# eggeek/distributed-oracle-search

Measured on AMD Instinct MI355X. Metric: CPD build sources/sec + GTEPS; table-search queries/sec; % HBM roofline, higher is better.
Workload: dtype u32

## Files before the change

distributed-oracle-search_amd/cpd.py:

```python
from __future__ import annotations

import ctypes as C
import os

import numpy as np

_HERE = os.path.dirname(os.path.abspath(__file__))
LIB_PATH = os.environ.get("CPD_LIB") or os.path.join(_HERE, "libcpd.so")

CPD_OK = 0
CPD_E_ARG = -1
CPD_E_HIP = -2
CPD_E_OOM = -3
CPD_E_NOROW = -4
CPD_E_RANGE = -5
CPD_E_IO = -6
PART_DIV = 0
PART_MOD = 1
INF = 0xFFFFFFFF
FM_ALL = 0xFFFF
MAX_WEIGHT_SETS = 8
MAX_LOAD_SLICES = 8
LOADS_ACCUMULATE = 1
TIMED_LOADS = 2
# ... 9 lines not shown
    "cpd_debug_rows", "cpd_index_create", "cpd_index_from_rows", "cpd_index_set_weights",
    "cpd_query_batch", "cpd_query_prepare", "cpd_query_run", "cpd_query_fetch",
    "cpd_index_free", "cpd_timing_enable", "cpd_timing_reset", "cpd_timing_get",
    "cpd_index_set_mode", "cpd_index_get_mode", "cpd_plan_cache", "cpd_index_create_empty",
    "cpd_index_append_rows", "cpd_index_append_built_rows", "cpd_index_info",
    "cpd_synth_road_graph_ex", "cpd_query_search", "cpd_query_search_counters",
    "cpd_graph_set_coords", "cpd_host_alloc", "cpd_host_free",
    "cpd_rows_lanes", "cpd_graph_hint_next", "cpd_graph_set_hbm_reserve",
    "cpd_device_mem_info", "cpd_rows_move_words", "cpd_rows_export_moves",
    "cpd_index_append_moves", "cpd_device_arena", "cpd_device_arena_release", "cpd_batch_bytes",
    "cpd_rows_move_bits", "cpd_graph_move_bits", "cpd_bucket_bytes", "cpd_space_check",
    "cpd_query_paths", "cpd_query_paths_fetch", "cpd_query_search_paths",
    "cpd_index_set_weight_sets", "cpd_query_costs", "cpd_query_costs_fetch",
    "cpd_query_loads", "cpd_query_loads_fetch", "cpd_query_loads_clear", "cpd_query_search_loads",
    "cpd_query_timed", "cpd_query_timed_fetch",
]
SYNTH_STYLES = {"shuffled": 7, "spec": 0}
INDEX_MODES = {"auto": 0, "rle": 1, "dense": 2}
SEARCH_FORMS = {"auto": 0, "tables": 1, "walks": 2}


class CpdError(RuntimeError):
    def __init__(self, code: int, msg: str):
        super().__init__(f"libcpd error {code}: {msg}")
        self.code = code


class PlanOpts(C.Structure):
    _fields_ = [("threads", C.c_int), ("witness_settle", C.c_uint32), ("verbose", C.c_int),
                ("no_hierarchy", C.c_int), ("ch_gpu", C.c_int), ("ch_device", C.c_int)]
# ... 153 lines not shown


class RoadGraph:

    def __init__(self, row_ptr, dst, w, x=None, y=None):
        self.row_ptr, self.dst, self.w = _u32(row_ptr), _u32(dst), _u32(w)
        self.x, self.y = x, y

    @property
    def n(self) -> int:
        return len(self.row_ptr) - 1

    @property
    def m(self) -> int:
        return len(self.dst)


def synth_road_graph(width: int, height: int, seed: int, mean_outdeg: float = 2.5,
                     style: str = "shuffled") -> RoadGraph:
    flags = SYNTH_STYLES[style]
    n, m = C.c_uint32(), C.c_uint32()
    _check(lib.cpd_synth_road_graph_ex(width, height, C.c_double(mean_outdeg), C.c_uint64(seed),
                                       C.c_uint32(flags), C.byref(n), C.byref(m), None, None,
                                       None, None, None))
    rp = np.empty(n.value + 1, np.uint32)
    dst = np.empty(m.value, np.uint32)
    w = np.empty(m.value, np.uint32)
    x = np.empty(n.value, np.int32)
    y = np.empty(n.value, np.int32)
    _check(lib.cpd_synth_road_graph_ex(width, height, C.c_double(mean_outdeg), C.c_uint64(seed),
# ... 190 lines not shown

    def move_bits(self) -> int:
        b = C.c_uint32()
        _check(lib.cpd_graph_move_bits(self._h, C.byref(b)))
        return b.value

    def set_coords(self, x, y) -> None:
        if x is None or y is None:
            _check(lib.cpd_graph_set_coords(self._h, None, None))
            return
        xs = np.ascontiguousarray(x, dtype=np.int32)
        ys = np.ascontiguousarray(y, dtype=np.int32)
        if len(xs) != self.plan.info()["n"] or len(ys) != len(xs):
            raise ValueError("coordinates must have one entry per node")
        _check(lib.cpd_graph_set_coords(self._h, _ptr(xs, i32p), _ptr(ys, i32p)))

    def build_rows(self, targets, reuse: Rows | None = None) -> Rows:
        t = _u32(targets)
        h = C.c_void_p()
        _check(lib.cpd_build_rows(self._h, _ptr(t, u32p), C.c_uint32(len(t)),
                                  reuse._h if reuse else None, C.byref(h)))
        if reuse is not None:
            return reuse
        return Rows(h)

    def hint_next(self, targets) -> None:
        t = _u32(targets)
        _check(lib.cpd_graph_hint_next(self._h, _ptr(t, u32p), C.c_uint32(len(t))))

    def debug_rows(self, targets, want_dist=True, want_fm=True):
# ... 363 lines not shown
```

distributed-oracle-search_amd/csrc/cpd_gpu_internal.hpp:

```cpp
#pragma once
#include <hip/hip_runtime_api.h>

#include <algorithm>
#include <array>
#include <cstring>
#include <functional>
#include <map>
#include <memory>
#include <mutex>
#include <string>
#include <vector>

#include "cpd_internal.hpp"
#include "cpd_kernels.hpp"
#include "cpd_switches.hpp"

#define HIP_CHECK(expr)                                                          \
    do {                                                                         \
        hipError_t _e = (expr);                                                  \
        if (_e != hipSuccess)                                                    \
            throw ::cpd::Error(_e == hipErrorOutOfMemory ? CPD_E_OOM : CPD_E_HIP, \
                               std::string(#expr) + ": " + hipGetErrorString(_e)); \
    } while (0)

namespace cpd {

struct ArenaScope {
    ArenaScope();
    ~ArenaScope();
    ArenaScope(const ArenaScope&) = delete;
// ... 131 lines not shown
    uint32_t acquire_set() {
        const uint32_t x = cur;
        cur = (cur + 1u) % nsets;
        if (emit_pending[x]) {
            HIP_CHECK(hipStreamWaitEvent(stream, ev_emit[x], 0));
            emit_pending[x] = false;
        }
        return x;
    }
    void drain_emits() {
        if (estream) HIP_CHECK(hipStreamSynchronize(estream));
        for (auto& p : emit_pending) p = false;
    }
    bool leaf_fm = false;
    DevBuf<uint32_t> leafbits;
    DevBuf<uint16_t> fmleaf;
    bool narrow = false;
    static constexpr uint32_t kNarrowProbe = 2;
    uint32_t narrow_probe = kNarrowProbe;
    HostBuf<uint32_t> ovf_hb;
    uint32_t ovf_h() const { return ovf_hb.p ? ovf_hb.p[0] : 0u; }
    DevBuf<uint16_t> d16;
    DevBuf<uint32_t> dbase, ovf, pool;
    uint32_t pool_cap = 0;
    NarrowRows narrow_rows(bool on) {
        if (!on) return NarrowRows{nullptr, nullptr, n, nullptr, nullptr, 0};
        return NarrowRows{d16.p, dbase.p, n, ovf.p, pool.p, pool_cap};
    }
    double n_leaf = 0, m_leaf = 0;
    std::vector<double> dsc_lvl_leaves;
// ... 17 lines not shown
    hipStream_t ustream = nullptr;
    hipEvent_t ev_up = nullptr, ev_down = nullptr, ev_fm[2] = {nullptr, nullptr};
    bool prepped = false;
    uint32_t prep_slot = 0;
    std::vector<uint32_t> prep_targets, hint;
    void drop_prep() {
        if (ustream) HIP_CHECK(hipStreamSynchronize(ustream));
        prepped = false;
    }
    DevBuf<uint32_t> asc_lvl_of, dsc_lvl_of;
    std::vector<uint32_t> up_item_first;
    DevBuf<uint32_t> up_items, up_init_slots;
    uint32_t n_init_slots = 0;
    std::vector<uint32_t> lane_key;
    DevBuf<uint32_t> seg_order;
    bool timing = false;
    std::vector<hipEvent_t> ev_pool;
    std::vector<Pending> pending;
    std::map<std::string, Agg> agg;

    ~cpd_graph();

    hipEvent_t get_event() {
        if (ev_pool.empty()) {
            hipEvent_t e;
            HIP_CHECK(hipEventCreate(&e));
            return e;
        }
        hipEvent_t e = ev_pool.back();
        ev_pool.pop_back();
// ... 190 lines not shown
```

distributed-oracle-search_amd/csrc/cpd_graph.cpp:

```cpp
#include <cmath>
#include <thread>

#include "cpd_gpu_internal.hpp"

namespace {

uint64_t pool_rows(uint32_t n, uint32_t B) {
    return std::max<uint64_t>((uint64_t)n * (B / 256u) / 8u, 4ull * n);
}

double batch_bytes_per_row(uint32_t n, uint32_t n_up, uint32_t npad, uint32_t fmb, bool narrow,
                           bool leaf_fm, uint32_t mbits) {
    const double rle = rle_fused(fmb) ? 12.0 * rle_emit_chunks(npad)
                                      : 3.0 * 5.0 / 32.0 * npad +
                                            (fmb == 4 ? 12.0 * rle_count_chunks(npad) : 0.0);
    const double fin = narrow ? (2.0 + 4.0 / 256.0 + 0.5) * n : 4.0 * n;
    return fin + 8.0 * n_up + 3.0 * fmb / 8.0 * npad + rle + (leaf_fm ? 0.5 * n : 0.0) +
           2.0 * mbits / 8.0 * npad;
}

std::vector<uint32_t> level_order(const cpd_plan& p, const std::vector<uint32_t>& level,
                                  uint32_t nlev, std::vector<uint32_t>& lvl_first) {
    const uint32_t n = p.n;
    std::vector<uint32_t> cnt(nlev + 1, 0);
// ... 179 lines not shown
        g.bytes += p.bytes;
        for (auto& f : p.late) g.bytes += f();
        ev_pool.push_back(p.a);
        ev_pool.push_back(p.b);
    }
    pending.swap(keep);
}

void cpd_graph::reserve_batch(uint32_t want) {
    ArenaScope carve;
    if (want == 0) {
        size_t free_b = 0, total_b = 0;
        HIP_CHECK(hipMemGetInfo(&free_b, &total_b));
        const double per = batch_bytes_per_row(n, n_up, npad, fmb, narrow, leaf_fm,
                                               1u << tlb);
        const double fixed = narrow ? 4096.0 * n : 0.0;
        const double avail = free_b > hbm_reserve + fixed ? (double)free_b - hbm_reserve - fixed
                                                          : 0.0;
        const double fit = 0.85 * avail / per;
        CPD_REQUIRE(hbm_reserve == 0 || fit >= 1024.0, CPD_E_OOM,
                    "HBM reserve of " + std::to_string(hbm_reserve >> 20) + " MiB leaves " +
                        std::to_string((size_t)avail >> 20) + " MiB: too little for a 1024-row batch");
        want = (uint32_t)std::min((double)switches().batch_max, std::max(1024.0, std::floor(fit / 1024) * 1024));
    }
    want = (want + 1023u) / 1024u * 1024u;
    if (want == B && upx[0].p) return;
    drain_emits();
    drop_prep();
    B = want;
    for (int s = 0; s < 2; ++s) {
        upx[s].alloc(std::max<size_t>((size_t)n_up * B, 1));
// ... 227 lines not shown
    g->dsc_desc.upload(desc.data(), desc.size(), g->stream);
}

void mark_leaves(cpd_graph* g, const cpd_plan* p) {
    std::vector<uint32_t> lb(g->npad / 32u, 0u);
    g->dsc_lvl_leaves.assign(g->dsc_lvl.size(), 0.0);
    for (uint32_t v = 0; v < g->n; ++v)
        if (p->ch.level_up[v] == 0) {
            const uint32_t c = p->order[v];
            lb[c >> 5] |= 1u << (c & 31u);
            g->n_leaf += 1;
            g->m_leaf += p->row_ptr[v + 1] - p->row_ptr[v];
            g->dsc_lvl_leaves[p->ch.level_dn[v]] += 1;
        }
    g->leafbits.upload(lb.data(), lb.size(), g->stream);
}

void chunk_narrow_up_levels(cpd_graph* g) {
    constexpr uint32_t kNarrow = 1024u;
    const uint32_t C = sweep_chunk_arcs();
    std::vector<uint32_t> items, slots;
    g->up_item_first.assign(g->asc_lvl.size(), 0);
    for (size_t l = 0; l + 1 < g->asc_lvl.size(); ++l) {
        g->up_item_first[l] = (uint32_t)(items.size() / 4);
        const uint32_t s0 = g->asc_lvl[l], s1 = g->asc_lvl[l + 1];
        if (l < 2 || s1 - s0 > kNarrow) continue;
        for (uint32_t x = s0; x < s1; ++x) {
            slots.push_back(x);
            for (uint32_t a = g->asc_off_host[x]; a < g->asc_off_host[x + 1]; a += C)
                items.insert(items.end(),
// ... 22 lines not shown

}

extern "C" {

int cpd_batch_bytes(uint32_t n, uint32_t max_degree, uint32_t batch, uint64_t* bytes) {
    return guarded([&] {
        CPD_REQUIRE(bytes && batch % 1024u == 0 && batch > 0, CPD_E_ARG,
                    "batch_bytes: batch must be a positive multiple of 1024");
        uint32_t shift = 0;
        while ((1u << shift) < std::max(1u, max_degree)) ++shift;
        const uint32_t fmb = fm_bits(shift);
        const uint32_t npad = (n + kFmTile - 1u) / kFmTile * kFmTile;
        const uint32_t mbits = max_degree <= 2u ? 1u : max_degree <= 4u ? 2u : 4u;
        *bytes = (uint64_t)(batch_bytes_per_row(n, n, npad, fmb, true, fmb == 4, mbits) * batch) +
                 (uint64_t)batch * (n / 256u + 1u) * 4u + 4096ull * n + 512ull * n + (64ull << 20);
    });
}

int cpd_graph_create(const cpd_plan* p, int device, cpd_graph** out) {
    return guarded([&] {
        CPD_REQUIRE(p && out, CPD_E_ARG, "graph: null argument");
        *out = nullptr;
        require_device();
        const double tg0 = now_seconds();
        auto g = std::make_unique<cpd_graph>();
        g->device = device;
        g->select();
        create_streams(g.get());
        trace_step("streams", tg0);
        column_space_csr(g.get(), p);
// ... 33 lines not shown
        g->reserve_batch(batch);
    });
}

int cpd_graph_set_hbm_reserve(cpd_graph* g, uint64_t bytes) {
    return guarded([&] {
        CPD_REQUIRE(g, CPD_E_ARG, "null graph");
        g->hbm_reserve = bytes;
    });
}

int cpd_graph_set_coords(cpd_graph* g, const int32_t* x, const int32_t* y) {
    return guarded([&] {
        CPD_REQUIRE(g, CPD_E_ARG, "null graph");
        if (!x || !y) {
            g->lane_key.clear();
            g->seg_order.release();
            return;
        }
        g->lane_key = hilbert_keys(x, y, g->n);
        if (switches().fm_order) {
            const uint32_t nseg = g->npad / 32u;
            std::vector<uint32_t> node_of(g->n);
            for (uint32_t v = 0; v < g->n; ++v) node_of[g->order[v]] = v;
            std::vector<uint64_t> kv(nseg);
            for (uint32_t sg = 0; sg < nseg; ++sg) {
                const uint32_t c = std::min(g->n - 1u, sg * 32u + 16u);
                kv[sg] = ((uint64_t)g->lane_key[node_of[c]] << 32) | sg;
            }
            std::sort(kv.begin(), kv.end());
            std::vector<uint32_t> so(nseg);
            for (uint32_t i = 0; i < nseg; ++i) so[i] = (uint32_t)kv[i];
            g->select();
            g->seg_order.upload(so.data(), nseg, g->stream);
            HIP_CHECK(hipStreamSynchronize(g->stream));
        }
    });
}

int cpd_graph_move_bits(const cpd_graph* g, uint32_t* bits) {
    return guarded([&] {
        CPD_REQUIRE(g && bits, CPD_E_ARG, "null argument");
        *bits = g->move_bits;
    });
}

int cpd_graph_get_batch(const cpd_graph* g, uint32_t* batch) {
    return guarded([&] {
        CPD_REQUIRE(g && batch, CPD_E_ARG, "null argument");
        *batch = g->B;
    });
// ... 46 lines not shown
```

distributed-oracle-search_amd/csrc/cpd_kernels.hip:

```cpp
#include <hip/hip_ext.h>
#include <hip/hip_runtime.h>
#include <hipcub/hipcub.hpp>
#include <algorithm>
#include <cstdint>
#include <type_traits>

#include "cpd_kernels.hpp"
#include "cpd_switches.hpp"

namespace cpd {
namespace kern {

constexpr uint32_t INF = 0xFFFFFFFFu;
constexpr uint32_t kNoEdge = 0xFFFFFFFFu;

__device__ __forceinline__ uint32_t sat_add(uint32_t d, uint32_t w) {
    uint32_t s = d + w;
    return (s < d) ? INF : s;
}

#ifndef CPD_RLE_LOOKBACK
#define CPD_RLE_LOOKBACK 16
#endif
constexpr uint32_t kSeg = 32;
// ... 858 lines not shown
    for (int cg = 0; cg < NC; cg += G) {
        if (cg + G < NC) issue(nxt, cg + G);
        finish(cur, cg);
        if ((cg + G) % 8 == 0) {
            const int wi = (cg + G) / 8 - 1;
#pragma unroll
            for (int i = 0; i < 4; ++i) fm_stage[(threadIdx.x * 4u + (uint32_t)i) * 4u + wi] = pk[i][wi];
        }
        cur = nxt;
    }
    uint4* __restrict__ o = reinterpret_cast<uint4*>(fm) + fm4_piece(4u * l4, nseg, cb / kSeg);
    const uint4* st = reinterpret_cast<const uint4*>(fm_stage) + threadIdx.x * 4u;
#pragma unroll
    for (int i = 0; i < 4; ++i) o[i] = st[i];
    }
}

template <int FMB>
__device__ __forceinline__ void seg_pass(const uint32_t (&v)[FmFmt<FMB>::kWords], uint32_t c0,
                                         uint32_t& h, uint32_t& S, uint32_t& cnt) {
    using F = FmFmt<FMB>;
#pragma unroll
    for (int k = 0; k < 32; ++k) {
        const uint32_t f = (v[k / F::kPer] >> (FMB * (k % F::kPer))) & F::kAll;
        const bool brk = (S & f) == 0u;
        cnt += brk ? 1u : 0u;
        h = brk ? c0 + (uint32_t)k : h;
        S = brk ? f : (S & f);
    }
}
// ... 3340 lines not shown
    switch (shift) {
        case 0: launch(kern::first_moves<1, 4, NARROW>, grid, blk, s, adj, dist, tgt, B, n, npad, r, fm, leafbits, fmleaf, nr); break;
        case 1: launch(kern::first_moves<2, 2, NARROW>, grid, blk, s, adj, dist, tgt, B, n, npad, r, fm, leafbits, fmleaf, nr); break;
        case 2:
            if constexpr (!NARROW) launch(kern::first_moves<4, 2, false>, grid, blk, s, adj, dist, tgt, B, n, npad, r, fm, leafbits, fmleaf, nr);
            break;
        case 3: launch(kern::first_moves<8, 1, NARROW>, grid, blk, s, adj, dist, tgt, B, n, npad, r, fm, leafbits, fmleaf, nr); break;
        default: launch(kern::first_moves<16, 1, NARROW>, grid, blk, s, adj, dist, tgt, B, n, npad, r, fm, leafbits, fmleaf, nr); break;
    }
}

void launch_first_moves(const uint32_t* adj32, uint32_t shift, const uint32_t* dist,
                        const uint32_t* tgt, uint32_t B, uint32_t rows, uint32_t n,
                        uint32_t npad, uint32_t* fm, const uint32_t* leafbits,
                        const uint16_t* fmleaf, NarrowRows nr, hipStream_t s,
                        const uint32_t* seg_order) {
    constexpr uint32_t tpb = 64u * kFmWpb;
    const dim3 grid((npad / kern::kSeg) * ((rows + 1023u) / 1024u) * (256u / tpb)), blk(tpb);
    const uint2* adj = reinterpret_cast<const uint2*>(adj32);
    if (nr.d16 && shift == 2)
        launch_shm(kern::first_moves_n4<2>, dim3(grid.x / kFmSpw), blk, 64u * tpb, s, adj, dist,
                   tgt, B, n, npad, xcd_remap(), fm, leafbits, fmleaf, nr, seg_order, kFmSpw);
    else if (nr.d16)
        launch_first_moves_t<true>(adj, shift, dist, tgt, B, n, npad, fm, leafbits, fmleaf, nr,
                                   grid, blk, s);
    else
        launch_first_moves_t<false>(adj, shift, dist, tgt, B, n, npad, fm, leafbits, fmleaf, nr,
                                    grid, blk, s);
}

bool first_moves_reads_own(uint32_t shift, bool narrow) {
    return !(narrow && shift == 2);
}

void launch_rle_count(const uint32_t* fm, uint32_t fmb, uint32_t npad, uint32_t nrows,
// ... 627 lines not shown
```

distributed-oracle-search_amd/csrc/cpd_kernels.hpp:

```cpp
#pragma once
#include <hip/hip_runtime_api.h>
#include <cstdint>

namespace cpd {

void set_launch_events(hipEvent_t start, hipEvent_t stop);

struct NarrowRows {
    uint16_t* d16;
    uint32_t* base;
    uint32_t n;
    uint32_t* ovf;
    uint32_t* pool;
    uint32_t cap;
};


constexpr uint32_t kLeafBit = 0x80000000u;
constexpr uint32_t kL1Bit = 0x40000000u;

void launch_sweep(bool ascend, const uint32_t* nodes, const uint32_t* arc_off,
                  const uint32_t* arcs , uint32_t slot0,
                  uint32_t count, uint32_t* dist, uint32_t* up, uint32_t ubase,
                  const uint32_t* uidx, const uint32_t* tgt, uint32_t B, uint32_t slabs,
// ... 11 lines not shown
                            const uint32_t* tgt, uint32_t B, uint32_t slabs,
                            const uint32_t* asc_nodes, const uint32_t* asc_off,
                            const uint32_t* asc_arcs, uint32_t* live, const uint32_t* tmask,
                            hipStream_t s);
uint32_t sweep_chunk_arcs();

void launch_target_mask(const uint32_t* tgt, uint32_t B, uint32_t* tmask, hipStream_t s);

void launch_live_stats(bool ascend, const uint32_t* nodes, const uint32_t* arc_off,
                       const uint32_t* arcs, const uint32_t* lvl_of, uint32_t slot0,
                       uint32_t slot1, uint32_t ubase, const uint32_t* uidx,
                       const uint32_t* live, unsigned int* stat, hipStream_t s);

uint32_t fm_bits(uint32_t shift);

void launch_first_moves(const uint32_t* adj, uint32_t shift, const uint32_t* dist,
                        const uint32_t* tgt, uint32_t B, uint32_t rows, uint32_t n,
                        uint32_t npad, uint32_t* fm, const uint32_t* leafbits,
                        const uint16_t* fmleaf, NarrowRows nr, hipStream_t s,
                        const uint32_t* seg_order = nullptr);
bool first_moves_reads_own(uint32_t shift, bool narrow);

constexpr uint32_t kFmTile = 2048;

void launch_rle_count(const uint32_t* fm, uint32_t fmb, uint32_t npad, uint32_t nrows,
                      uint32_t* counts, uint32_t* st, uint8_t* rc, hipStream_t s,
                      const uint32_t* gate = nullptr);

void launch_rle_moves(const uint32_t* fm, uint32_t fmb, uint32_t npad, uint32_t nrows,
                      const uint32_t* st, const uint8_t* rc, const uint32_t* out_row,
                      uint32_t lb, uint32_t* dense, hipStream_t s);
uint32_t rle_emit_chunks(uint32_t npad);
void launch_rle_emit(const uint32_t* fm, uint32_t npad, uint32_t nrows, const uint32_t* out_row,
                     uint32_t lb, uint32_t* dense, uint32_t* xe, uint32_t* xs, uint32_t* cc,
                     uint32_t* counts, hipStream_t s);
// ... 161 lines not shown
```

distributed-oracle-search_amd/csrc/cpd_rows.cpp:

```cpp
#include "cpd_gpu_internal.hpp"

void cpd_rows::settle() const {
    std::lock_guard<std::mutex> l(settle_mu);
    HIP_CHECK(hipSetDevice(device));
    wait();
    for (auto& b : retired) spare.push_back(std::move(b));
    retired.clear();
    if (pending.empty()) return;
    for (auto& b : pending) {
        for (uint32_t i = 0; i < b->k; ++i)
            offsets.push_back(offsets.back() + b->counts.p[b->pos_of[i]]);
        spare.push_back(std::move(b));
    }
    pending.clear();
    total = offsets.back();
    hipStream_t st = thread_stream(device);
    off.upload(offsets.data(), offsets.size(), st);
    HIP_CHECK(hipStreamSynchronize(st));
}

cpd_rows::Batch* cpd_rows::new_batch(uint32_t B) {
    for (size_t i = 0; i < retired.size();) {
        if (hipEventQuery(retired[i]->ev) == hipSuccess) {
            spare.push_back(std::move(retired[i]));
// ... 162 lines not shown

void launch_fm(cpd_graph* g, uint32_t k, bool narrow, uint32_t* fm, uint32_t slot) {
    const uint32_t B = g->B, n = g->n;
    const NarrowRows nr = g->narrow_rows(narrow);
    const double drow = narrow ? 2.0 + 4.0 / 256.0 : 4.0;
    const uint32_t fslabs = (k + 1023u) / 1024u;
    const double nl = g->leaf_fm ? g->n_leaf : 0.0, ml = g->leaf_fm ? g->m_leaf : 0.0;
    const double own = first_moves_reads_own(g->adj_shift, narrow) ? drow * (n - nl) : 0.0;
    double fbytes =
        (own + drow * (g->m - ml) + 0.5 * nl + g->fmb / 8.0 * g->npad) *
            (fslabs * 1024.0) +
        8.0 * (double)(n - nl) * (double)(1u << g->adj_shift) * fslabs + 4.0 * g->npad / 32.0;
    g->timed("first_moves", fbytes, [&] {
        launch_first_moves(g->adj.p, g->adj_shift, g->dist.p, g->fm_tgt.p, B, k, n, g->npad,
                           fm, g->leaf_fm ? g->leafbits.p : nullptr,
                           g->leaf_fm ? g->fmleaf.p : nullptr, nr, g->stream, g->seg_order.p);
    });
    HIP_CHECK(hipEventRecord(g->ev_fm[slot], g->stream));
}

void launch_down_fm(cpd_graph* g, uint32_t k, bool narrow, uint32_t* fm, uint32_t slot) {
    launch_down(g, k, narrow, slot);
    launch_fm(g, k, narrow, fm, slot);
}

void prepare_targets(cpd_graph* g, const uint32_t* targets, uint32_t k, uint32_t slot) {
    auto& S = g->bs[slot];
    CPD_REQUIRE(g->has_ch, CPD_E_ARG,
                "graph was created from a plan without hierarchy: it can serve queries "
                "but not build rows");
    std::vector<uint32_t> cols(g->B), idx(k);
// ... 491 lines not shown
```

distributed-oracle-search_amd/csrc/cpd_switches.cpp:

```cpp
#include "cpd_switches.hpp"

#include <algorithm>
#include <cstdio>
#include <cstdlib>

namespace cpd {
namespace {

bool env_on(const char* name) {
    const char* e = std::getenv(name);
    return !(e && *e == '0');
}
bool env_set(const char* name) {
    const char* e = std::getenv(name);
    return e && *e && *e != '0';
}

Switches read_switches() {
    Switches s;
    s.live = env_on("CPD_LIVE");
    s.sort = env_on("CPD_SORT");
    s.lane_key = env_on("CPD_LANE_KEY");
    s.xcd = env_on("CPD_XCD");
    s.async = env_on("CPD_ASYNC");
// ... 6 lines not shown
    s.batch_max = (uint32_t)std::max(1024ul, std::min(32768ul, b / 1024ul * 1024ul));
    s.trace = env_set("CPD_TRACE");
    s.search_trace = env_set("CPD_SEARCH_TRACE");
    return s;
}

}

const Switches& switches() {
    static const Switches s = read_switches();
    return s;
}

bool narrow_rows_on() { return env_on("CPD_NARROW"); }

uint64_t search_pool_words(uint64_t words) {
    const char* e = std::getenv("CPD_SEARCH_POOL_WORDS");
    return e && *e ? std::min<uint64_t>(words, std::strtoull(e, nullptr, 10)) : words;
}

ChPrio ch_prio() {
    ChPrio p;
    if (const char* e = std::getenv("CPD_CH_PRIO")) {
        long a, b, c;
        if (std::sscanf(e, "%ld,%ld,%ld", &a, &b, &c) == 3) p = {a, b, c};
    }
    return p;
}

}
// ... 1 lines not shown
```

distributed-oracle-search_amd/csrc/cpd_switches.hpp:

```cpp
#pragma once
#include <cstdint>

namespace cpd {

struct Switches {
    bool live;
    bool sort;
    bool lane_key;
    bool xcd;
    bool async;
    bool rle_fused;
    bool leaffm;
    bool overlap;
    bool fm_order;
    uint32_t batch_max;
    bool trace;
    bool search_trace;
};
const Switches& switches();

bool narrow_rows_on();

uint64_t search_pool_words(uint64_t words);

struct ChPrio {
    int64_t ed = 8, deleted = 2, depth = 12;
};
ChPrio ch_prio();

}
```

include/cpd_api.h:

```cpp
#ifndef CPD_API_H
#define CPD_API_H

#include <stdint.h>
#include <stddef.h>

#ifdef __cplusplus
extern "C" {
#endif

#define CPD_OK          0
#define CPD_E_ARG      -1
#define CPD_E_HIP      -2
#define CPD_E_OOM      -3
#define CPD_E_NOROW    -4
#define CPD_E_RANGE    -5
#define CPD_E_IO       -6

#define CPD_PART_DIV    0
#define CPD_PART_MOD    1

#define CPD_MAX_DEGREE 15u
#define CPD_INF        0xFFFFFFFFu
#define CPD_FM_ALL     0xFFFFu

// ... 67 lines not shown
                    const uint32_t* w, uint32_t n, uint32_t m, const cpd_plan_opts* opts,
                    cpd_plan** out, int* status);
void cpd_plan_free(cpd_plan* p);

int  cpd_device_count(int* count);
int  cpd_device_mem_info(int device, uint64_t* free_bytes, uint64_t* total_bytes);
int  cpd_device_arena(int device, uint64_t bytes, int touch);
int  cpd_device_arena_release(int device);
int  cpd_batch_bytes(uint32_t n, uint32_t max_degree, uint32_t batch, uint64_t* bytes);
int  cpd_graph_create(const cpd_plan* p, int device, cpd_graph** out);
int  cpd_graph_set_batch(cpd_graph* g, uint32_t batch);
int  cpd_graph_get_batch(const cpd_graph* g, uint32_t* batch);
int  cpd_graph_move_bits(const cpd_graph* g, uint32_t* bits);
int  cpd_graph_set_hbm_reserve(cpd_graph* g, uint64_t bytes);
int  cpd_graph_set_coords(cpd_graph* g, const int32_t* x, const int32_t* y);
void cpd_graph_free(cpd_graph* g);

int  cpd_build_rows(cpd_graph* g, const uint32_t* targets, uint32_t ntargets,
                    cpd_rows* reuse, cpd_rows** out);
int  cpd_graph_hint_next(cpd_graph* g, const uint32_t* targets, uint32_t ntargets);
int  cpd_rows_count(const cpd_rows* r, uint32_t* nrows, uint64_t* total_runs);
int  cpd_rows_export(const cpd_rows* r, uint64_t* offsets ,
                     uint32_t* runs );
int  cpd_rows_export_range(const cpd_rows* r, uint32_t first, uint32_t count,
                           uint64_t* offsets , uint32_t* runs);
int  cpd_rows_move_words(const cpd_rows* r, uint32_t* words);
int  cpd_rows_move_bits(const cpd_rows* r, uint32_t* bits);
int  cpd_rows_export_moves(const cpd_rows* r, uint32_t first, uint32_t count,
                           uint32_t* moves );
int  cpd_rows_targets(const cpd_rows* r, uint32_t* targets );
// ... 147 lines not shown
```

Before: 443,000.

## Stage shared neighbour distance rows in LDS via precomputed first-move patch plans

Adds a host-built patch plan that groups spatially ordered 32-column segments into patches whose distinct neighbour rows fit in LDS. A new first-moves kernel loads those rows, the edge weights, index tables and leaf first-moves into LDS once per patch and strip, then computes argmin first moves from LDS. The aim is to avoid re-reading the same neighbour distance rows from HBM for every column. In exchange it costs host-side plan construction, extra device memory for plan tables and large LDS use per workgroup, which limits occupancy. It only runs on the narrow, coordinate-ordered path.

```diff
diff --git a/distributed-oracle-search_amd/cpd.py b/distributed-oracle-search_amd/cpd.py
--- a/distributed-oracle-search_amd/cpd.py
+++ b/distributed-oracle-search_amd/cpd.py
@@ -47,6 +47,7 @@
     "cpd_index_set_weight_sets", "cpd_query_costs", "cpd_query_costs_fetch",
     "cpd_query_loads", "cpd_query_loads_fetch", "cpd_query_loads_clear", "cpd_query_search_loads",
     "cpd_query_timed", "cpd_query_timed_fetch",
+    "cpd_graph_fm_patch_info", "cpd_graph_set_fm_patch_capacity", "cpd_fm_patch_plan",
 ]
 SYNTH_STYLES = {"shuffled": 7, "spec": 0}
 INDEX_MODES = {"auto": 0, "rle": 1, "dense": 2}
@@ -230,6 +231,27 @@
     @property
     def m(self) -> int:
         return len(self.dst)
+
+
+def fm_patch_plan(row_ptr, dst, leafbits=None, seg_order=None, segs: int = 4, strip: int = 256,
+                  capacity: int = 80 * 1024) -> dict:
+    rp, d = _u32(row_ptr), _u32(dst)
+    n = len(rp) - 1
+    nseg = (n + 2047) // 2048 * 64
+    lb = None if leafbits is None else _u32(leafbits)
+    so = None if seg_order is None else _u32(seg_order)
+    if (lb is not None and len(lb) != nseg) or (so is not None and len(so) != nseg):
+        raise ValueError("leafbits and seg_order have one entry per 32-column segment")
+    args = (_ptr(rp, u32p), _ptr(d, u32p), C.c_uint32(n), _ptr(lb, u32p), _ptr(so, u32p),
+            C.c_uint32(segs), C.c_uint32(strip), C.c_uint32(capacity))
+    npatch, nstage = C.c_uint32(), C.c_uint32()
+    _check(lib.cpd_fm_patch_plan(*args, C.byref(npatch), C.byref(nstage), None, None, None))
+    desc = np.empty((npatch.value, 4), np.uint32)
+    stage = np.empty(nstage.value, np.uint32)
+    idx = np.empty((nseg, 32, 4), np.uint16)
+    _check(lib.cpd_fm_patch_plan(*args, C.byref(npatch), C.byref(nstage), _ptr(desc, u32p),
+                                 _ptr(stage, u32p), _ptr(idx, u16p)))
+    return {"desc": desc, "stage": stage, "idx": idx}
 
 
 def synth_road_graph(width: int, height: int, seed: int, mean_outdeg: float = 2.5,
@@ -450,6 +472,14 @@
         if len(xs) != self.plan.info()["n"] or len(ys) != len(xs):
             raise ValueError("coordinates must have one entry per node")
         _check(lib.cpd_graph_set_coords(self._h, _ptr(xs, i32p), _ptr(ys, i32p)))
+
+    def fm_patch_info(self) -> dict:
+        p, r, c = C.c_uint32(), C.c_uint32(), C.c_uint32()
+        _check(lib.cpd_graph_fm_patch_info(self._h, C.byref(p), C.byref(r), C.byref(c)))
+        return {"patches": p.value, "stage_rows": r.value, "capacity": c.value}
+
+    def set_fm_patch_capacity(self, nbytes: int) -> None:
+        _check(lib.cpd_graph_set_fm_patch_capacity(self._h, C.c_uint32(nbytes)))
 
     def build_rows(self, targets, reuse: Rows | None = None) -> Rows:
         t = _u32(targets)
diff --git a/distributed-oracle-search_amd/csrc/cpd_gpu_internal.hpp b/distributed-oracle-search_amd/csrc/cpd_gpu_internal.hpp
--- a/distributed-oracle-search_amd/csrc/cpd_gpu_internal.hpp
+++ b/distributed-oracle-search_amd/csrc/cpd_gpu_internal.hpp
@@ -14,6 +14,7 @@
 #include "cpd_internal.hpp"
 #include "cpd_kernels.hpp"
 #include "cpd_switches.hpp"
+#include "fm_patch_plan.hpp"
 
 #define HIP_CHECK(expr)                                                          \
     do {                                                                         \
@@ -175,6 +176,7 @@
     }
     bool leaf_fm = false;
     DevBuf<uint32_t> leafbits;
+    std::vector<uint32_t> leafbits_host;
     DevBuf<uint16_t> fmleaf;
     bool narrow = false;
     static constexpr uint32_t kNarrowProbe = 2;
@@ -222,6 +224,14 @@
     uint32_t n_init_slots = 0;
     std::vector<uint32_t> lane_key;
     DevBuf<uint32_t> seg_order;
+    std::vector<uint32_t> seg_order_host;
+    DevBuf<uint32_t> fm_patch_desc, fm_patch_stage;
+    DevBuf<uint16_t> fm_patch_idx;
+    uint32_t fm_patch_n = 0, fm_patch_rows = 0, fm_patch_cap = 0;
+    void build_fm_patch(uint32_t cap_bytes);
+    FmPatchDev fm_patch() const {
+        return FmPatchDev{fm_patch_desc.p, fm_patch_stage.p, fm_patch_idx.p, fm_patch_n};
+    }
     bool timing = false;
     std::vector<hipEvent_t> ev_pool;
     std::vector<Pending> pending;
diff --git a/distributed-oracle-search_amd/csrc/cpd_graph.cpp b/distributed-oracle-search_amd/csrc/cpd_graph.cpp
--- a/distributed-oracle-search_amd/csrc/cpd_graph.cpp
+++ b/distributed-oracle-search_amd/csrc/cpd_graph.cpp
@@ -217,7 +217,8 @@
         HIP_CHECK(hipMemGetInfo(&free_b, &total_b));
         const double per = batch_bytes_per_row(n, n_up, npad, fmb, narrow, leaf_fm,
                                                1u << tlb);
-        const double fixed = narrow ? 4096.0 * n : 0.0;
+        const double fixed =
+            narrow ? 4096.0 * n + (adj_shift == 2 ? (double)fm_patch_plan_bytes(n, npad) : 0.0) : 0.0;
         const double avail = free_b > hbm_reserve + fixed ? (double)free_b - hbm_reserve - fixed
                                                           : 0.0;
         const double fit = 0.85 * avail / per;
@@ -475,6 +476,7 @@
             g->dsc_lvl_leaves[p->ch.level_dn[v]] += 1;
         }
     g->leafbits.upload(lb.data(), lb.size(), g->stream);
+    g->leafbits_host = std::move(lb);
 }
 
 void chunk_narrow_up_levels(cpd_graph* g) {
@@ -527,7 +529,8 @@
         const uint32_t npad = (n + kFmTile - 1u) / kFmTile * kFmTile;
         const uint32_t mbits = max_degree <= 2u ? 1u : max_degree <= 4u ? 2u : 4u;
         *bytes = (uint64_t)(batch_bytes_per_row(n, n, npad, fmb, true, fmb == 4, mbits) * batch) +
-                 (uint64_t)batch * (n / 256u + 1u) * 4u + 4096ull * n + 512ull * n + (64ull << 20);
+                 (uint64_t)batch * (n / 256u + 1u) * 4u + 4096ull * n + 512ull * n + (64ull << 20) +
+                 (fmb == 4 ? fm_patch_plan_bytes(n, npad) : 0ull);
     });
 }
 
@@ -591,8 +594,12 @@
     return guarded([&] {
         CPD_REQUIRE(g, CPD_E_ARG, "null graph");
         if (!x || !y) {
+            g->select();
+            HIP_CHECK(hipStreamSynchronize(g->stream));
             g->lane_key.clear();
             g->seg_order.release();
+            g->seg_order_host.clear();
+            g->build_fm_patch(0);
             return;
         }
         g->lane_key = hilbert_keys(x, y, g->n);
@@ -609,9 +616,81 @@
             std::vector<uint32_t> so(nseg);
             for (uint32_t i = 0; i < nseg; ++i) so[i] = (uint32_t)kv[i];
             g->select();
+            HIP_CHECK(hipStreamSynchronize(g->stream));
             g->seg_order.upload(so.data(), nseg, g->stream);
             HIP_CHECK(hipStreamSynchronize(g->stream));
-        }
+            g->seg_order_host = std::move(so);
+            g->build_fm_patch(kFmPatchLds);
+        }
+    });
+}
+
+void cpd_graph::build_fm_patch(uint32_t cap_bytes) {
+    fm_patch_desc.release();
+    fm_patch_stage.release();
+    fm_patch_idx.release();
+    fm_patch_n = fm_patch_rows = fm_patch_cap = 0;
+    if (!cap_bytes || seg_order_host.empty() || !has_ch || !narrow || adj_shift != 2 ||
+        !fm_patch_on())
+        return;
+    FmPatchPlan plan = build_fm_patch_plan(
+        rowc_host.data(), dst_col_host.data(), n, npad, leaf_fm ? leafbits_host.data() : nullptr,
+        seg_order_host.data(), kFmPatchSegs, kFmPatchStrip, cap_bytes);
+    fm_patch_rows = (uint32_t)plan.stage.size();
+    if (plan.stage.empty()) plan.stage.push_back(0u);
+    fm_patch_desc.upload(plan.desc.data(), plan.desc.size(), stream);
+    fm_patch_stage.upload(plan.stage.data(), plan.stage.size(), stream);
+    fm_patch_idx.upload(plan.idx.data(), plan.idx.size(), stream);
+    HIP_CHECK(hipStreamSynchronize(stream));
+    fm_patch_n = plan.npatch();
+    fm_patch_cap = cap_bytes;
+}
+
+int cpd_graph_set_fm_patch_capacity(cpd_graph* g, uint32_t bytes) {
+    return guarded([&] {
+        CPD_REQUIRE(g, CPD_E_ARG, "null graph");
+        CPD_REQUIRE(bytes <= kFmPatchLds, CPD_E_ARG,
+                    "patch capacity above the kernel's " + std::to_string(kFmPatchLds) + " B of LDS");
+        g->select();
+        HIP_CHECK(hipStreamSynchronize(g->stream));
+        try {
+            g->build_fm_patch(bytes ? bytes : kFmPatchLds);
+        } catch (const std::invalid_argument& e) {
+            g->build_fm_patch(kFmPatchLds);
+            throw Error(CPD_E_ARG, e.what());
+        }
+    });
+}
+
+int cpd_graph_fm_patch_info(const cpd_graph* g, uint32_t* patches, uint32_t* stage_rows,
+                            uint32_t* capacity) {
+    return guarded([&] {
+        CPD_REQUIRE(g && patches && stage_rows && capacity, CPD_E_ARG, "null argument");
+        *patches = g->fm_patch_n;
+        *stage_rows = g->fm_patch_rows;
+        *capacity = g->fm_patch_cap;
+    });
+}
+
+int cpd_fm_patch_plan(const uint32_t* row_ptr, const uint32_t* dst, uint32_t n,
+                      const uint32_t* leafbits, const uint32_t* seg_order, uint32_t segs,
+                      uint32_t strip, uint32_t capacity, uint32_t* patches, uint32_t* stage_rows,
+                      uint32_t* desc, uint32_t* stage, uint16_t* idx) {
+    return guarded([&] {
+        CPD_REQUIRE(row_ptr && patches && stage_rows, CPD_E_ARG, "patch plan: null argument");
+        const uint32_t npad = (n + kFmTile - 1u) / kFmTile * kFmTile;
+        FmPatchPlan plan;
+        try {
+            plan = build_fm_patch_plan(row_ptr, dst, n, npad, leafbits, seg_order, segs, strip,
+                                       capacity);
+        } catch (const std::invalid_argument& e) {
+            throw Error(CPD_E_ARG, e.what());
+        }
+        *patches = plan.npatch();
+        *stage_rows = (uint32_t)plan.stage.size();
+        if (desc) std::copy(plan.desc.begin(), plan.desc.end(), desc);
+        if (stage) std::copy(plan.stage.begin(), plan.stage.end(), stage);
+        if (idx) std::copy(plan.idx.begin(), plan.idx.end(), idx);
     });
 }
 
diff --git a/distributed-oracle-search_amd/csrc/cpd_kernels.hip b/distributed-oracle-search_amd/csrc/cpd_kernels.hip
--- a/distributed-oracle-search_amd/csrc/cpd_kernels.hip
+++ b/distributed-oracle-search_amd/csrc/cpd_kernels.hip
@@ -7,6 +7,7 @@
 
 #include "cpd_kernels.hpp"
 #include "cpd_switches.hpp"
+#include "fm_patch_plan.hpp"
 
 namespace cpd {
 namespace kern {
@@ -896,6 +897,150 @@
 #pragma unroll
     for (int i = 0; i < 4; ++i) o[i] = st[i];
     }
+}
+
+template <int P, int S>
+__global__ __launch_bounds__(P * S / 4) void first_moves_patch(
+    const uint2* __restrict__ adj, const uint32_t* __restrict__ tgt, uint32_t B, uint32_t n,
+    uint32_t npad, uint32_t remap, uint32_t* __restrict__ fm,
+    const uint32_t* __restrict__ leafbits, const uint16_t* __restrict__ fmleaf, NarrowRows nr,
+    const uint32_t* __restrict__ seg_order, const uint4* __restrict__ pdesc,
+    const uint32_t* __restrict__ pstage, const uint16_t* __restrict__ pidx, uint32_t npatch) {
+    static_assert(S == 128 || S == 256, "a strip is a half or a whole 256-target group");
+    constexpr uint32_t T = P * S / 4;
+    constexpr uint32_t LS = S / 4;
+    constexpr uint32_t RP = S / 8;
+    constexpr uint32_t LP = S / 32;
+    static_assert(T % 64 == 0 && P * 16 <= T, "workgroup shape");
+    extern __shared__ uint4 fmp_lds[];
+    const uint32_t nseg = npad / kSeg;
+    const uint32_t L = remap ? xcd_block(blockIdx.x, gridDim.x) : blockIdx.x;
+    const uint32_t strip = L / npatch, patch = L - strip * npatch;
+    const uint4 pd = pdesc[patch];
+    const uint32_t pos0 = pd.x, cnt = pd.y, nst = pd.w;
+    const uint32_t* __restrict__ stage = pstage + pd.z;
+    const uint32_t t = threadIdx.x;
+    const uint32_t grp = strip * (uint32_t)S / 256u;
+    const uint32_t B8 = B / 8u, B32 = B / 32u;
+
+    uint4* const l_idx4 = fmp_lds;
+    uint32_t* const l_w = reinterpret_cast<uint32_t*>(fmp_lds + P * 16);
+    uint4* const l_rows = fmp_lds + fm_patch_tab_bytes(P) / 16u;
+    uint32_t* const l_base =
+        reinterpret_cast<uint32_t*>(fmp_lds + fm_patch_base_off(P, S, nst) / 16u);
+    uint4* const l_leaf = fmp_lds + fm_patch_leaf_off(P, S, nst) / 16u;
+
+    uint32_t segs[P], lbs[P];
+#pragma unroll
+    for (int i = 0; i < P; ++i) {
+        const bool in = (uint32_t)i < cnt;
+        segs[i] = in ? (seg_order ? seg_order[pos0 + i] : pos0 + i) : 0u;
+        lbs[i] = in && leafbits ? leafbits[segs[i]] : 0u;
+    }
+
+    if (t < cnt * 16u) l_idx4[t] = reinterpret_cast<const uint4*>(pidx)[(size_t)pos0 * 16u + t];
+#pragma unroll
+    for (uint32_t j0 = 0; j0 < P * 128u; j0 += T) {
+        const uint32_t j = j0 + t, i = j >> 7, e = j & 127u;
+        uint32_t sg = 0;
+#pragma unroll
+        for (int ii = 0; ii < P; ++ii) sg = (uint32_t)ii == i ? segs[ii] : sg;
+        if (i < cnt) l_w[j] = sg * kSeg + e / 4u < n ? adj[(size_t)sg * 128u + e].y : 0u;
+    }
+#pragma unroll
+    for (uint32_t j0 = 0; j0 < P * 32u * LP; j0 += T) {
+        const uint32_t j = j0 + t, piece = j % LP, cc = (j / LP) & 31u, i = j / (32u * LP);
+        uint32_t sg = 0, lb = 0, lbase = 0;
+#pragma unroll
+        for (int ii = 0; ii < P; ++ii) {
+            sg = (uint32_t)ii == i ? segs[ii] : sg;
+            lb = (uint32_t)ii == i ? lbs[ii] : lb;
+            lbase += (uint32_t)ii < i ? __popc(lbs[ii]) : 0u;
+        }
+        if ((lb >> cc) & 1u) {
+            const uint32_t slot = lbase + __popc(lb & ((1u << cc) - 1u));
+            l_leaf[slot * LP + piece] = reinterpret_cast<const uint4*>(
+                fmleaf)[(size_t)(sg * kSeg + cc) * B32 + strip * LP + piece];
+        }
+    }
+    for (uint32_t r = t; r < nst; r += T) l_base[r] = nr.base[(size_t)grp * nr.n + stage[r]];
+    {
+        constexpr int U = 8;
+        constexpr uint32_t RPP = T / RP;
+        const uint32_t rin = t / RP, piece = t % RP;
+        const uint4* __restrict__ d16v = reinterpret_cast<const uint4*>(nr.d16) + strip * RP + piece;
+        for (uint32_t r0 = rin; r0 < nst; r0 += U * RPP) {
+            uint4 v[U];
+#pragma unroll
+            for (int u = 0; u < U; ++u) {
+                const uint32_t r = r0 + (uint32_t)u * RPP;
+                v[u] = r < nst ? d16v[(size_t)stage[r] * B8] : make_uint4(0u, 0u, 0u, 0u);
+            }
+#pragma unroll
+            for (int u = 0; u < U; ++u) {
+                const uint32_t r = r0 + (uint32_t)u * RPP;
+                if (r < nst) l_rows[r * RP + piece] = v[u];
+            }
+        }
+    }
+    __syncthreads();
+
+    const uint32_t si = t / LS, li = t % LS;
+    if (si >= cnt) return;
+    uint32_t seg = 0, lb = 0, lbase = 0;
+#pragma unroll
+    for (int ii = 0; ii < P; ++ii) {
+        seg = (uint32_t)ii == si ? segs[ii] : seg;
+        lb = (uint32_t)ii == si ? lbs[ii] : lb;
+        lbase += (uint32_t)ii < si ? __popc(lbs[ii]) : 0u;
+    }
+    const uint32_t cb = seg * kSeg;
+    const uint32_t l4 = strip * LS + li;
+    const uint4 tc = reinterpret_cast<const uint4*>(tgt)[l4];
+    const uint2* const l_iq = reinterpret_cast<const uint2*>(l_idx4) + si * 32u;
+    const uint4* const l_wq = reinterpret_cast<const uint4*>(l_w) + si * 32u;
+    const uint2* const l_q = reinterpret_cast<const uint2*>(l_rows) + li;
+    const uint16_t* const l_lf = reinterpret_cast<const uint16_t*>(l_leaf) + li;
+    uint32_t pk[4][4];
+#pragma unroll
+    for (int p = 0; p < 4; ++p) pk[0][p] = pk[1][p] = pk[2][p] = pk[3][p] = 0xFFFFFFFFu;
+#pragma unroll
+    for (int cc = 0; cc < (int)kSeg; ++cc) {
+        const uint32_t c = cb + (uint32_t)cc;
+        if (c >= n) continue;
+        uint32_t bits;
+        if ((lb >> cc) & 1u) {
+            bits = l_lf[(lbase + __popc(lb & ((1u << cc) - 1u))) * LS];
+        } else {
+            const uint2 iq = l_iq[cc];
+            const uint4 wq = l_wq[cc];
+            const uint32_t id[4] = {iq.x & 0xFFFFu, iq.x >> 16, iq.y & 0xFFFFu, iq.y >> 16};
+            const uint32_t w[4] = {wq.x, wq.y, wq.z, wq.w};
+            uint4 dn = make_uint4(INF, INF, INF, INF);
+            bits = 0;
+#pragma unroll
+            for (int k = 0; k < 4; ++k) {
+                if (id[k] == 0xFFFFu) continue;
+                const uint4 dv = nl_finish(NLoad{l_base[id[k]], l_q[id[k] * LS]}, nr, l4);
+                argmin_fold<0>(dn.x, bits, sat_add(dv.x, w[k]), k);
+                argmin_fold<1>(dn.y, bits, sat_add(dv.y, w[k]), k);
+                argmin_fold<2>(dn.z, bits, sat_add(dv.z, w[k]), k);
+                argmin_fold<3>(dn.w, bits, sat_add(dv.w, w[k]), k);
+            }
+            bits = fm_wild4(tc, dn, c, bits);
+        }
+        const uint32_t f0 = bits & 0xFu, f1 = (bits >> 4) & 0xFu;
+        const uint32_t f2 = (bits >> 8) & 0xFu, f3 = (bits >> 12) & 0xFu;
+        const int wi = cc / 8, sh = 4 * (cc % 8);
+        const uint32_t keep = ~(0xFu << sh);
+        pk[0][wi] = (pk[0][wi] & keep) | (f0 << sh);
+        pk[1][wi] = (pk[1][wi] & keep) | (f1 << sh);
+        pk[2][wi] = (pk[2][wi] & keep) | (f2 << sh);
+        pk[3][wi] = (pk[3][wi] & keep) | (f3 << sh);
+    }
+    uint4* __restrict__ o = reinterpret_cast<uint4*>(fm) + fm4_piece(4u * l4, nseg, seg);
+#pragma unroll
+    for (int i = 0; i < 4; ++i) o[i] = make_uint4(pk[i][0], pk[i][1], pk[i][2], pk[i][3]);
 }
 
 template <int FMB>
@@ -4266,11 +4411,20 @@
                         const uint32_t* tgt, uint32_t B, uint32_t rows, uint32_t n,
                         uint32_t npad, uint32_t* fm, const uint32_t* leafbits,
                         const uint16_t* fmleaf, NarrowRows nr, hipStream_t s,
-                        const uint32_t* seg_order) {
+                        const uint32_t* seg_order, FmPatchDev fp) {
     constexpr uint32_t tpb = 64u * kFmWpb;
     const dim3 grid((npad / kern::kSeg) * ((rows + 1023u) / 1024u) * (256u / tpb)), blk(tpb);
     const uint2* adj = reinterpret_cast<const uint2*>(adj32);
-    if (nr.d16 && shift == 2)
+    if (nr.d16 && shift == 2 && fp.npatch) {
+        constexpr uint32_t P = kFmPatchSegs, S = kFmPatchStrip;
+        auto kernel = kern::first_moves_patch<(int)P, (int)S>;
+        (void)hipFuncSetAttribute(reinterpret_cast<const void*>(kernel),
+                                  hipFuncAttributeMaxDynamicSharedMemorySize, (int)kFmPatchLds);
+        const uint32_t strips = (rows + 1023u) / 1024u * (1024u / S);
+        launch_shm(kernel, dim3(fp.npatch * strips), dim3(P * S / 4u), kFmPatchLds, s, adj, tgt, B,
+                   n, npad, xcd_remap(), fm, leafbits, fmleaf, nr, seg_order,
+                   reinterpret_cast<const uint4*>(fp.desc), fp.stage, fp.idx, fp.npatch);
+    } else if (nr.d16 && shift == 2)
         launch_shm(kern::first_moves_n4<2>, dim3(grid.x / kFmSpw), blk, 64u * tpb, s, adj, dist,
                    tgt, B, n, npad, xcd_remap(), fm, leafbits, fmleaf, nr, seg_order, kFmSpw);
     else if (nr.d16)
diff --git a/distributed-oracle-search_amd/csrc/cpd_kernels.hpp b/distributed-oracle-search_amd/csrc/cpd_kernels.hpp
--- a/distributed-oracle-search_amd/csrc/cpd_kernels.hpp
+++ b/distributed-oracle-search_amd/csrc/cpd_kernels.hpp
@@ -49,11 +49,17 @@
 
 uint32_t fm_bits(uint32_t shift);
 
+struct FmPatchDev {
+    const uint32_t* desc = nullptr;
+    const uint32_t* stage = nullptr;
+    const uint16_t* idx = nullptr;
+    uint32_t npatch = 0;
+};
 void launch_first_moves(const uint32_t* adj, uint32_t shift, const uint32_t* dist,
                         const uint32_t* tgt, uint32_t B, uint32_t rows, uint32_t n,
                         uint32_t npad, uint32_t* fm, const uint32_t* leafbits,
                         const uint16_t* fmleaf, NarrowRows nr, hipStream_t s,
-                        const uint32_t* seg_order = nullptr);
+                        const uint32_t* seg_order = nullptr, FmPatchDev patch = {});
 bool first_moves_reads_own(uint32_t shift, bool narrow);
 
 constexpr uint32_t kFmTile = 2048;
diff --git a/distributed-oracle-search_amd/csrc/cpd_rows.cpp b/distributed-oracle-search_amd/csrc/cpd_rows.cpp
--- a/distributed-oracle-search_amd/csrc/cpd_rows.cpp
+++ b/distributed-oracle-search_amd/csrc/cpd_rows.cpp
@@ -200,7 +200,8 @@
     g->timed("first_moves", fbytes, [&] {
         launch_first_moves(g->adj.p, g->adj_shift, g->dist.p, g->fm_tgt.p, B, k, n, g->npad,
                            fm, g->leaf_fm ? g->leafbits.p : nullptr,
-                           g->leaf_fm ? g->fmleaf.p : nullptr, nr, g->stream, g->seg_order.p);
+                           g->leaf_fm ? g->fmleaf.p : nullptr, nr, g->stream, g->seg_order.p,
+                           g->fm_patch());
     });
     HIP_CHECK(hipEventRecord(g->ev_fm[slot], g->stream));
 }
diff --git a/distributed-oracle-search_amd/csrc/cpd_switches.cpp b/distributed-oracle-search_amd/csrc/cpd_switches.cpp
--- a/distributed-oracle-search_amd/csrc/cpd_switches.cpp
+++ b/distributed-oracle-search_amd/csrc/cpd_switches.cpp
@@ -44,6 +44,8 @@
 
 bool narrow_rows_on() { return env_on("CPD_NARROW"); }
 
+bool fm_patch_on() { return env_set("CPD_FM_PATCH"); }
+
 uint64_t search_pool_words(uint64_t words) {
     const char* e = std::getenv("CPD_SEARCH_POOL_WORDS");
     return e && *e ? std::min<uint64_t>(words, std::strtoull(e, nullptr, 10)) : words;
diff --git a/distributed-oracle-search_amd/csrc/cpd_switches.hpp b/distributed-oracle-search_amd/csrc/cpd_switches.hpp
--- a/distributed-oracle-search_amd/csrc/cpd_switches.hpp
+++ b/distributed-oracle-search_amd/csrc/cpd_switches.hpp
@@ -21,6 +21,8 @@
 
 bool narrow_rows_on();
 
+bool fm_patch_on();
+
 uint64_t search_pool_words(uint64_t words);
 
 struct ChPrio {
diff --git a/distributed-oracle-search_amd/csrc/fm_patch_plan.cpp b/distributed-oracle-search_amd/csrc/fm_patch_plan.cpp
--- /dev/null
+++ b/distributed-oracle-search_amd/csrc/fm_patch_plan.cpp
@@ -0,0 +1,105 @@
+#include "fm_patch_plan.hpp"
+
+#include <algorithm>
+#include <stdexcept>
+#include <string>
+
+namespace cpd {
+namespace {
+
+void segment_needs(const uint32_t* row_ptr, const uint32_t* dst, uint32_t n,
+                   const uint32_t* leafbits, uint32_t seg, std::vector<uint32_t>& cols,
+                   uint32_t& nleaf) {
+    const uint32_t lb = leafbits ? leafbits[seg] : 0u;
+    for (uint32_t cc = 0; cc < 32u; ++cc) {
+        const uint32_t c = seg * 32u + cc;
+        if (c >= n) break;
+        if ((lb >> cc) & 1u) {
+            ++nleaf;
+            continue;
+        }
+        for (uint32_t e = row_ptr[c]; e < row_ptr[c + 1]; ++e) cols.push_back(dst[e]);
+    }
+}
+
+void sort_unique(std::vector<uint32_t>& v) {
+    std::sort(v.begin(), v.end());
+    v.erase(std::unique(v.begin(), v.end()), v.end());
+}
+
+}
+
+FmPatchPlan build_fm_patch_plan(const uint32_t* row_ptr, const uint32_t* dst, uint32_t n,
+                                uint32_t npad, const uint32_t* leafbits,
+                                const uint32_t* seg_order, uint32_t P, uint32_t S,
+                                uint32_t cap_bytes) {
+    if (!row_ptr || (!dst && n && row_ptr[n]) || npad % 32u || npad < n || !P || P > 64u ||
+        !S || S % 32u)
+        throw std::invalid_argument("patch plan: inconsistent arguments");
+    const uint32_t nseg = npad / 32u;
+    for (uint32_t c = 0; c < n; ++c) {
+        if (row_ptr[c + 1] < row_ptr[c] || row_ptr[c + 1] - row_ptr[c] > 4u)
+            throw std::invalid_argument("patch plan: out-degree above 4");
+        for (uint32_t e = row_ptr[c]; e < row_ptr[c + 1]; ++e)
+            if (dst[e] >= n) throw std::invalid_argument("patch plan: edge head out of range");
+    }
+    if (seg_order) {
+        std::vector<uint8_t> seen(nseg, 0);
+        for (uint32_t i = 0; i < nseg; ++i) {
+            if (seg_order[i] >= nseg || seen[seg_order[i]])
+                throw std::invalid_argument("patch plan: segment order is no permutation");
+            seen[seg_order[i]] = 1;
+        }
+    }
+    auto seg_at = [&](uint32_t pos) { return seg_order ? seg_order[pos] : pos; };
+
+    FmPatchPlan plan;
+    plan.idx.assign((size_t)nseg * 128u, kFmPatchNone);
+    std::vector<uint32_t> cur, cand;
+    for (uint32_t p0 = 0; p0 < nseg; p0 += P) {
+        const uint32_t p1 = std::min(nseg, p0 + P);
+        uint32_t s = p0;
+        while (s < p1) {
+            cur.clear();
+            uint32_t cnt = 0, nleaf = 0;
+            while (s + cnt < p1) {
+                cand = cur;
+                uint32_t nl = nleaf;
+                segment_needs(row_ptr, dst, n, leafbits, seg_at(s + cnt), cand, nl);
+                sort_unique(cand);
+                if (cand.size() >= kFmPatchNone ||
+                    fm_patch_lds_bytes(P, S, (uint32_t)cand.size(), nl) > cap_bytes) {
+                    if (cnt == 0)
+                        throw std::invalid_argument(
+                            "patch plan: one segment needs " +
+                            std::to_string(fm_patch_lds_bytes(P, S, (uint32_t)cand.size(), nl)) +
+                            " B of LDS, capacity " + std::to_string(cap_bytes));
+                    break;
+                }
+                cur.swap(cand);
+                nleaf = nl;
+                ++cnt;
+            }
+            const uint32_t off = (uint32_t)plan.stage.size();
+            plan.desc.insert(plan.desc.end(), {s, cnt, off, (uint32_t)cur.size()});
+            plan.stage.insert(plan.stage.end(), cur.begin(), cur.end());
+            for (uint32_t i = 0; i < cnt; ++i) {
+                const uint32_t seg = seg_at(s + i);
+                const uint32_t lb = leafbits ? leafbits[seg] : 0u;
+                for (uint32_t cc = 0; cc < 32u && seg * 32u + cc < n; ++cc) {
+                    if ((lb >> cc) & 1u) continue;
+                    const uint32_t c = seg * 32u + cc;
+                    for (uint32_t e = row_ptr[c]; e < row_ptr[c + 1]; ++e) {
+                        const auto it = std::lower_bound(cur.begin(), cur.end(), dst[e]);
+                        plan.idx[((size_t)(s + i) * 32u + cc) * 4u + (e - row_ptr[c])] =
+                            (uint16_t)(it - cur.begin());
+                    }
+                }
+            }
+            s += cnt;
+        }
+    }
+    return plan;
+}
+
+}
diff --git a/distributed-oracle-search_amd/csrc/fm_patch_plan.hpp b/distributed-oracle-search_amd/csrc/fm_patch_plan.hpp
--- /dev/null
+++ b/distributed-oracle-search_amd/csrc/fm_patch_plan.hpp
@@ -0,0 +1,42 @@
+#pragma once
+#include <cstddef>
+#include <cstdint>
+#include <vector>
+
+namespace cpd {
+
+constexpr uint32_t kFmPatchSegs = 4;
+constexpr uint32_t kFmPatchStrip = 256;
+constexpr uint32_t kFmPatchLds = 80u * 1024u;
+
+constexpr uint16_t kFmPatchNone = 0xFFFFu;
+
+constexpr uint32_t fm_patch_tab_bytes(uint32_t P) { return P * 128u * (2u + 4u); }
+constexpr uint32_t fm_patch_base_off(uint32_t P, uint32_t S, uint32_t nstage) {
+    return fm_patch_tab_bytes(P) + nstage * S * 2u;
+}
+constexpr uint32_t fm_patch_leaf_off(uint32_t P, uint32_t S, uint32_t nstage) {
+    return fm_patch_base_off(P, S, nstage) + (nstage * 4u + 15u) / 16u * 16u;
+}
+constexpr uint32_t fm_patch_lds_bytes(uint32_t P, uint32_t S, uint32_t nstage, uint32_t nleaf) {
+    return fm_patch_leaf_off(P, S, nstage) + nleaf * (S / 2u);
+}
+
+struct FmPatchPlan {
+    std::vector<uint32_t> desc;
+    std::vector<uint32_t> stage;
+    std::vector<uint16_t> idx;
+    uint32_t npatch() const { return (uint32_t)(desc.size() / 4u); }
+    size_t bytes() const { return desc.size() * 4u + stage.size() * 4u + idx.size() * 2u; }
+};
+
+constexpr uint64_t fm_patch_plan_bytes(uint32_t n, uint32_t npad) {
+    return 8ull * npad + 16ull * n + 16ull * (npad / 32u);
+}
+
+FmPatchPlan build_fm_patch_plan(const uint32_t* row_ptr, const uint32_t* dst, uint32_t n,
+                                uint32_t npad, const uint32_t* leafbits,
+                                const uint32_t* seg_order, uint32_t P, uint32_t S,
+                                uint32_t cap_bytes);
+
+}
diff --git a/include/cpd_api.h b/include/cpd_api.h
--- a/include/cpd_api.h
+++ b/include/cpd_api.h
@@ -105,6 +105,13 @@
 int  cpd_graph_move_bits(const cpd_graph* g, uint32_t* bits);
 int  cpd_graph_set_hbm_reserve(cpd_graph* g, uint64_t bytes);
 int  cpd_graph_set_coords(cpd_graph* g, const int32_t* x, const int32_t* y);
+int  cpd_graph_fm_patch_info(const cpd_graph* g, uint32_t* patches, uint32_t* stage_rows,
+                             uint32_t* capacity);
+int  cpd_graph_set_fm_patch_capacity(cpd_graph* g, uint32_t bytes);
+int  cpd_fm_patch_plan(const uint32_t* row_ptr, const uint32_t* dst, uint32_t n,
+                       const uint32_t* leafbits, const uint32_t* seg_order, uint32_t segs,
+                       uint32_t strip, uint32_t capacity, uint32_t* patches,
+                       uint32_t* stage_rows, uint32_t* desc, uint32_t* stage, uint16_t* idx);
 void cpd_graph_free(cpd_graph* g);
 
 int  cpd_build_rows(cpd_graph* g, const uint32_t* targets, uint32_t ntargets,
diff --git a/tools_scripts/fm_patch_model.py b/tools_scripts/fm_patch_model.py
--- /dev/null
+++ b/tools_scripts/fm_patch_model.py
@@ -0,0 +1,80 @@
+import os
+import sys
+import time
+
+import numpy as np
+
+ROOT = os.path.dirname(os.path.dirname(os.path.abspath(__file__)))
+sys.path[:0] = [os.path.join(ROOT, "distributed-oracle-search_amd")]
+import cpd
+
+
+def hilbert(x, y, bits=16):
+    x, y = x.astype(np.int64).copy(), y.astype(np.int64).copy()
+    d = np.zeros(len(x), np.int64)
+    s = 1 << (bits - 1)
+    while s:
+        rx, ry = (x & s) > 0, (y & s) > 0
+        d += s * s * ((3 * rx) ^ ry)
+        x &= s - 1
+        y &= s - 1
+        f = ~ry
+        sw = f & rx
+        x[sw], y[sw] = s - 1 - x[sw], s - 1 - y[sw]
+        x[f], y[f] = y[f].copy(), x[f].copy()
+        s >>= 1
+    return d
+
+
+def lds_bytes(P, S, nst, nleaf):
+    return P * 768 + nst * S * 2 + (nst * 4 + 15) // 16 * 16 + nleaf * (S // 2)
+
+
+side = int(sys.argv[1]) if len(sys.argv) > 1 else 1000
+rows = int(sys.argv[2]) if len(sys.argv) > 2 else 28672
+t0 = time.time()
+g = cpd.synth_road_graph(side, side, 1, style="shuffled")
+plan = cpd.Plan(g, threads=8)
+order = plan.order().astype(np.int64)
+n = g.n
+inv = np.empty(n, np.int64)
+inv[order] = np.arange(n)
+deg = np.diff(g.row_ptr.astype(np.int64))
+rp = np.zeros(n + 1, np.int64)
+rp[1:] = np.cumsum(deg[inv])
+src = np.repeat(np.arange(n), deg)
+eo = np.lexsort((np.arange(len(src)), order[src]))
+dst = order[g.dst[eo]].astype(np.uint32)
+nseg = (n + 2047) // 2048 * 64
+leafcol = np.zeros(nseg * 32, bool)
+leafcol[order[plan.export_ch()["level_up"] == 0]] = True
+lb = (leafcol.reshape(nseg, 32) * (1 << np.arange(32, dtype=np.uint64))).sum(1).astype(np.uint32)
+nleaf_seg = leafcol.reshape(nseg, 32).sum(1)
+mid = np.minimum(n - 1, np.arange(nseg) * 32 + 16)
+x, y = g.x[inv[mid]].astype(np.int64), g.y[inv[mid]].astype(np.int64)
+sc = max(int(x.max() - x.min()), int(y.max() - y.min()), 1)
+key = hilbert((x - x.min()) * 65535 // sc, (y - y.min()) * 65535 // sc)
+so = np.lexsort((np.arange(nseg), key)).astype(np.uint32)
+nonleaf = ~leafcol[:n]
+distinct = len(np.unique(dst[np.repeat(nonleaf, np.diff(rp))]))
+print(f"graph {n} nodes, {nonleaf.sum()} gathering columns, {distinct} distinct neighbour rows, "
+      f"{int(nleaf_seg.sum())} leaf columns ({time.time() - t0:.0f} s)", flush=True)
+rowb = 2.0 * rows + 4.0 * rows / 256
+print(f"distinct rows once: {distinct * rowb / 1e9:.1f} GB, leaf sets "
+      f"{nleaf_seg.sum() * 0.5 * rows / 1e9:.1f} GB")
+for P, S, cap in [(8, 128, 80), (4, 256, 80), (8, 128, 160), (4, 256, 160), (2, 256, 52),
+                  (2, 256, 80), (4, 128, 52), (8, 256, 160)]:
+    p = cpd.fm_patch_plan(rp.astype(np.uint32), dst, lb, so, segs=P, strip=S, capacity=cap * 1024)
+    d = p["desc"].astype(np.int64)
+    nst = d[:, 3]
+    cs = np.concatenate([[0], np.cumsum(nleaf_seg[so])])
+    nl = cs[d[:, 0] + d[:, 1]] - cs[d[:, 0]]
+    lds = np.array([lds_bytes(P, S, a, b) for a, b in zip(nst, nl)])
+    strips = rows / S
+    tables = (16 + 4 * nst + d[:, 1] * (256 + 1024 + 8)).sum() * strips
+    read = nst.sum() * rowb + nleaf_seg.sum() * 0.5 * rows + tables + 4.0 * rows * len(d) / S
+    print(f"P={P} S={S} cap={cap} KiB: {len(d)} sub-patches ({(d[:, 1] < P).mean() * 100:.0f}% "
+          f"short), stage rows mean {nst.mean():.1f} p99 {np.percentile(nst, 99):.0f} max "
+          f"{nst.max()}, staged/distinct {nst.sum() / distinct:.3f}, LDS mean "
+          f"{lds.mean() / 1024:.1f} max {lds.max() / 1024:.1f} KiB, {160 // cap} workgroups/CU, "
+          f"read {read / 1e9:.1f} GB per {rows}-row launch", flush=True)
```

Result: slower. 432,400 (-2.4%).
